# microsoft/ptgnn

Hardware: AMD Instinct MI355X
Metric: edges/sec per MP layer (higher is better)
Workload: dtype f32; 1 GPU; cfg3: Graph2Class-style batch, 48 graphs N=115772, T0=8->T=17, E=625130 (incl. reverse+self), Typilus GGNN arch: 8 GGNN layers H=128 (+concat residual), max; hidden=128, mode=forward (inference), fp32, plan_build_in_step=True, message_rows=shared per (edge type, source) pair, parallelism=single GPU, minibatches_rotated=4

## Files before the change

ptgnn_amd/csrc/stream_gemm.hip:

```cpp
#include <stdlib.h>

#include "dense_common.h"
#include <atomic>

#include "stream_gemm.h"

namespace ptgnn_amd {
namespace {

using u32x4 = __attribute__((ext_vector_type(4))) uint32_t;

constexpr int kLdsBudget = 160 * 1024;
constexpr size_t kEpiBytes = 16 + 8 * 8 * 36 * sizeof(float);

__device__ __forceinline__ f32x16 zero16() {
  f32x16 v;
#pragma unroll
  for (int r = 0; r < 16; ++r) v[r] = 0.f;
  return v;
}

struct ARows {
  const float *c0, *c1, *n0, *n1;
};

__device__ __forceinline__ float4 load_piece(const ARows &r, int cc, int ch0, int nch, int g) {
  const bool nx = cc >= nch;
  const int c = nx ? cc - nch : cc;
  const float *b0 = nx ? r.n0 : r.c0;
  const float *b1 = nx ? r.n1 : r.c1;
  const float *p = c < ch0 ? b0 + c * 32 : b1 + (c - ch0) * 32;
  return *reinterpret_cast<const float4 *>(p + g * 8);
}

__device__ __forceinline__ int lane_piece_offset(int hi) { return hi * 4; }

template <int NBLK, int NACC, int PH, bool GRU>
__device__ __forceinline__ void chunk_f32(f32x16 (&acc)[NACC], float4 (&buf)[4], float4 (&bcur)[NBLK],
                                          const float *bl, int cbs, int kofs, int kofs_next, const ARows &rows,
                                          int cnext, int ch0, int nch) {
#pragma unroll
  for (int g = 0; g < 4; ++g) {
    float4 bn[NBLK];
    const int ko = g < 3 ? kofs + (g + 1) * 8 : kofs_next;
#pragma unroll
    for (int n = 0; n < NBLK; ++n) bn[n] = *reinterpret_cast<const float4 *>(bl + n * cbs + ko);
    __builtin_amdgcn_sched_barrier(0);
    const float4 a = buf[g];
#define PTGNN_STEP(C)                                                                     \
    _Pragma("unroll") for (int n = 0; n < NBLK; ++n) {                                    \
      const int t = (GRU && PH == 1 && n == 2) ? 3 : n;                                   \
      acc[t] = __builtin_amdgcn_mfma_f32_32x32x2f32(a.C, bcur[n].C, acc[t], 0, 0, 0);     \
    }
    PTGNN_STEP(x) PTGNN_STEP(y) PTGNN_STEP(z) PTGNN_STEP(w)
#undef PTGNN_STEP
    __builtin_amdgcn_sched_barrier(0);
#pragma unroll
    for (int n = 0; n < NBLK; ++n) bcur[n] = bn[n];
  }
#pragma unroll
  for (int g = 0; g < 4; ++g) {
    buf[g] = load_piece(rows, cnext, ch0, nch, g);
    __builtin_amdgcn_sched_barrier(0);
  }
}

struct Slab {
  int ld;
  __device__ __forceinline__ Slab(int K, int ) { ld = K + 4; }
  static size_t bytes(int K, int rows) { return (size_t)rows * (K + 4) * 4; }

  __device__ __forceinline__ void put4(float *smem, int r, int k, float4 v) const {
    *reinterpret_cast<float4 *>(smem + r * ld + k) = v;
  }
};

template <int NT, typename SrcFn, typename LiveFn>
__device__ __forceinline__ void fill_slab(float *smem, const Slab &sl, int rows, int kq, SrcFn src, LiveFn live) {
  constexpr int UB = 8;
  const int total = rows * kq;
  for (int i0 = threadIdx.x; i0 < total; i0 += NT * UB) {
    float4 v[UB];
    int rr[UB], qq[UB];
#pragma unroll
    for (int u = 0; u < UB; ++u) {
      const int i = i0 + u * NT;
      const int ic = i < total ? i : total - 1;
      rr[u] = ic / kq;
      qq[u] = ic - rr[u] * kq;
    }
#pragma unroll
    for (int u = 0; u < UB; ++u) {
      v[u] = *reinterpret_cast<const float4 *>(src(rr[u], qq[u]));
      __builtin_amdgcn_sched_barrier(0);
    }
#pragma unroll
    for (int u = 0; u < UB; ++u) {
      if (i0 + u * NT < total) sl.put4(smem, rr[u], qq[u] * 4, live(rr[u]) ? v[u] : make_float4(0.f, 0.f, 0.f, 0.f));
    }
  }
}

template <int NBLK, int NACC, bool GRU>
__device__ __forceinline__ void unit_kloop(f32x16 (&acc)[NACC], float4 (&a0)[4], float4 (&a1)[4],
                                           const float *smem, const Slab &sl, int li, int hi,
                                           const ARows &rows, int ch0, int nch) {
  const float *bl = smem + li * sl.ld + hi * 4;
  const int cbs = 32 * sl.ld;
  const int e0 = GRU ? ch0 : nch;
  float4 bcur[NBLK];
#pragma unroll
  for (int n = 0; n < NBLK; ++n) bcur[n] = *reinterpret_cast<const float4 *>(bl + n * cbs);
  for (int c = 0; c < e0; c += 2) {
    const int kn = c + 2 < nch ? c * 32 + 64 : 0;
    chunk_f32<NBLK, NACC, 0, GRU>(acc, a0, bcur, bl, cbs, c * 32, c * 32 + 32, rows, c + 2, ch0, nch);
    chunk_f32<NBLK, NACC, 0, GRU>(acc, a1, bcur, bl, cbs, c * 32 + 32, kn, rows, c + 3, ch0, nch);
  }
  if constexpr (GRU) {
    for (int c = ch0; c < nch; c += 2) {
      const int kn = c + 2 < nch ? c * 32 + 64 : 0;
      chunk_f32<NBLK, NACC, 1, GRU>(acc, a0, bcur, bl, cbs, c * 32, c * 32 + 32, rows, c + 2, ch0, nch);
      chunk_f32<NBLK, NACC, 1, GRU>(acc, a1, bcur, bl, cbs, c * 32 + 32, kn, rows, c + 3, ch0, nch);
    }
  }
}

__device__ __forceinline__ void prologue_loads(float4 (&a0)[4], float4 (&a1)[4], const ARows &rows, int ch0,
                                               int nch) {
#pragma unroll
  for (int g = 0; g < 4; ++g) {
    a0[g] = load_piece(rows, 0, ch0, nch, g);
    __builtin_amdgcn_sched_barrier(0);
  }
#pragma unroll
  for (int g = 0; g < 4; ++g) {
    a1[g] = load_piece(rows, 1, ch0, nch, g);
    __builtin_amdgcn_sched_barrier(0);
  }
}

__device__ __forceinline__ void unit_fence() {
  __builtin_amdgcn_s_waitcnt(0x0F70);
  __builtin_amdgcn_sched_barrier(0);
}

__device__ __forceinline__ int claim_unit(int *counter) {
  int v = 0;
  if ((threadIdx.x & 63) == 0) v = atomicAdd(counter, 1);
  return __builtin_amdgcn_readfirstlane(v);
}

constexpr int kTqLd = 36;
constexpr int kTqFloats = 8 * kTqLd;

__device__ __forceinline__ float4 tq_transpose(float *tq, int lane, int li, int hi, float v0, float v1, float v2,
                                               float v3) {
  float *w = tq + (4 * hi) * kTqLd + li;
  w[0] = v0; w[kTqLd] = v1; w[2 * kTqLd] = v2; w[3 * kTqLd] = v3;
  __builtin_amdgcn_wave_barrier();
  const float4 o = *reinterpret_cast<const float4 *>(tq + (lane >> 3) * kTqLd + (lane & 7) * 4);
  __builtin_amdgcn_wave_barrier();
  return o;
}

__device__ __forceinline__ void tq_untranspose(float *tq, int lane, int li, int hi, float4 in, float (&v)[4]) {
  *reinterpret_cast<float4 *>(tq + (lane >> 3) * kTqLd + (lane & 7) * 4) = in;
  __builtin_amdgcn_wave_barrier();
  const float *r = tq + (4 * hi) * kTqLd + li;
  v[0] = r[0]; v[1] = r[kTqLd]; v[2] = r[2 * kTqLd]; v[3] = r[3 * kTqLd];
  __builtin_amdgcn_wave_barrier();
}

using u32x4 = __attribute__((ext_vector_type(4))) uint32_t;

__device__ __forceinline__ __amdgpu_buffer_rsrc_t rows_descriptor(float *base , int64_t ld, int64_t rows_left,
                                                                  int width ) {
  const uint64_t b = reinterpret_cast<uint64_t>(base);
  const uint32_t lo = __builtin_amdgcn_readfirstlane((uint32_t)b), hi = __builtin_amdgcn_readfirstlane((uint32_t)(b >> 32));
  const int64_t rows = rows_left < 32 ? rows_left : 32;
  const int64_t bytes = rows > 0 ? ((rows - 1) * ld + width) * 4 : 0;
  return __builtin_amdgcn_make_buffer_rsrc(reinterpret_cast<float *>(((uint64_t)hi << 32) | lo), 0,
                                           __builtin_amdgcn_readfirstlane((int)bytes), 0x00020000);
}

__device__ __forceinline__ void store_row4(__amdgpu_buffer_rsrc_t rsrc, int lane_bytes, int uniform_bytes, float4 o) {
  const u32x4 v = {__float_as_uint(o.x), __float_as_uint(o.y), __float_as_uint(o.z), __float_as_uint(o.w)};
  __builtin_amdgcn_raw_buffer_store_b128(v, rsrc, lane_bytes + uniform_bytes, 0, 0);
}

template <int ACT, bool BIAS = true>
__device__ __forceinline__ void store_block_tq(const f32x16 &c, float *tq, float *yblk ,
                                               int64_t ld_y, float bv, int64_t rows_left, int lane, int li, int hi,
                                               const float *addblk = nullptr, int64_t ld_add = 0) {
  auto val = [&](int r) { return BIAS ? act_apply<ACT>(c[r] + bv) : act_apply<ACT>(c[r]); };
  float4 addv[4];
  if (addblk) {
#pragma unroll
    for (int q = 0; q < 4; ++q) {
      int64_t r = 8 * q + (lane >> 3);
      r = r < rows_left ? r : rows_left - 1;
      addv[q] = *reinterpret_cast<const float4 *>(addblk + r * ld_add + (lane & 7) * 4);
    }
  }
#ifdef PTGNN_GLOBAL_STORES
  float *yp = yblk + (int64_t)(lane >> 3) * ld_y + (lane & 7) * 4;
#pragma unroll
  for (int q = 0; q < 4; ++q) {
    float4 o = tq_transpose(tq, lane, li, hi, val(4 * q), val(4 * q + 1), val(4 * q + 2), val(4 * q + 3));
    if (addblk) { o.x += addv[q].x; o.y += addv[q].y; o.z += addv[q].z; o.w += addv[q].w; }
    if (8 * q + (lane >> 3) < rows_left) *reinterpret_cast<float4 *>(yp + (int64_t)(8 * q) * ld_y) = o;
  }
#else
  const __amdgpu_buffer_rsrc_t rsrc = rows_descriptor(yblk, ld_y, rows_left, 32);
  const int ldb = (int)ld_y * 4;
  const int lane_bytes = (lane >> 3) * ldb + (lane & 7) * 16;
#pragma unroll
  for (int q = 0; q < 4; ++q) {
    float4 o = tq_transpose(tq, lane, li, hi, val(4 * q), val(4 * q + 1), val(4 * q + 2), val(4 * q + 3));
    if (addblk) { o.x += addv[q].x; o.y += addv[q].y; o.z += addv[q].z; o.w += addv[q].w; }
    store_row4(rsrc, lane_bytes, 8 * q * ldb, o);
  }
#endif
}

struct LinearArgs {
  const float *x; int64_t rows; int K; int64_t ld_x;
  const float *w; int n_out; const float *bias; int act;
  float *y; int64_t ld_y;
  const float *addend; int64_t ld_add;
  int nrb, ncs, rps, run_len;
  int lds_floats;
  int vec_store;
};

template <int ACT>
__device__ __forceinline__ void store_block(const f32x16 &c, float *yp, int64_t ld_y, float bv, int64_t row0,
                                            int64_t rows, int hi) {
  if (row0 + 32 <= rows) {
#pragma unroll
    for (int r = 0; r < 16; ++r)
      yp[(int64_t)((r & 3) + 8 * (r >> 2)) * ld_y] = act_apply<ACT>(c[r] + bv);
  } else {
#pragma unroll
    for (int r = 0; r < 16; ++r) {
      const int rr = (r & 3) + 8 * (r >> 2);
      if (row0 + rr + 4 * hi < rows) yp[(int64_t)rr * ld_y] = act_apply<ACT>(c[r] + bv);
    }
  }
}

template <int NB>
__device__ __forceinline__ void linear_epilogue(const LinearArgs &p, f32x16 (&acc)[NB], float *tq, int64_t row0,
                                                int col_base, int lane, int li, int hi) {
#pragma unroll
  for (int n = 0; n < NB; ++n) {
    const int col = col_base + n * 32 + li;
    if (col_base + n * 32 < p.n_out) {
      const float bv = p.bias ? p.bias[col] : 0.f;
      if (p.vec_store) {
        float *yb = p.y + row0 * p.ld_y + col_base + n * 32;
        const int64_t left = p.rows - row0;
        if (p.bias) {
#pragma unroll
          for (int r = 0; r < 16; ++r) acc[n][r] += bv;
        }
        const float *ab = p.addend ? p.addend + row0 * p.ld_add + col_base + n * 32 : nullptr;
        if (p.act == PTGNN_AMD_ACT_TANH) store_block_tq<PTGNN_AMD_ACT_TANH, false>(acc[n], tq, yb, p.ld_y, 0.f, left, lane, li, hi, ab, p.ld_add);
        else if (p.act == PTGNN_AMD_ACT_RELU) store_block_tq<PTGNN_AMD_ACT_RELU, false>(acc[n], tq, yb, p.ld_y, 0.f, left, lane, li, hi, ab, p.ld_add);
        else store_block_tq<PTGNN_AMD_ACT_NONE, false>(acc[n], tq, yb, p.ld_y, 0.f, left, lane, li, hi, ab, p.ld_add);
      } else {
        float *yp = p.y + (row0 + 4 * hi) * p.ld_y + col;
        if (p.act == PTGNN_AMD_ACT_TANH) store_block<PTGNN_AMD_ACT_TANH>(acc[n], yp, p.ld_y, bv, row0, p.rows, hi);
        else if (p.act == PTGNN_AMD_ACT_RELU) store_block<PTGNN_AMD_ACT_RELU>(acc[n], yp, p.ld_y, bv, row0, p.rows, hi);
        else store_block<PTGNN_AMD_ACT_NONE>(acc[n], yp, p.ld_y, bv, row0, p.rows, hi);
      }
    }
    acc[n] = zero16();
  }
}

template <int NB>
__global__ __launch_bounds__(512, 2) void k_stream_linear(LinearArgs p) {
  extern __shared__ __attribute__((aligned(16))) float smem[];
  constexpr int NT = 512, BN = 32 * NB;
  const int b = blockIdx.x, G = gridDim.x;
  int slab, part;
  if (G % (kNumXcd * p.ncs) == 0) {
    const int xcd = b % kNumXcd, j = b / kNumXcd;
    slab = j % p.ncs;
    part = xcd + kNumXcd * (j / p.ncs);
  } else {
    slab = b / p.rps;
    part = b % p.rps;
  }
  const int rb0 = part * p.run_len;
  const int rb1 = rb0 + p.run_len < p.nrb ? rb0 + p.run_len : p.nrb;
  if (rb0 >= rb1) return;
  const int count = rb1 - rb0;

  const Slab sl(p.K, BN);
  int *counter = reinterpret_cast<int *>(smem + p.lds_floats);
  float *const tq = smem + p.lds_floats + 4 + (threadIdx.x >> 6) * kTqFloats;
  if (threadIdx.x == 0) *counter = 0;
  const int col_base = slab * BN;
  fill_slab<NT>(smem, sl, BN, p.K >> 2,
                       [&](int r, int q) {
                         const int wr = col_base + r < p.n_out ? col_base + r : p.n_out - 1;
                         return p.w + (int64_t)wr * p.K + q * 4;
                       },
                       [&](int r) { return col_base + r < p.n_out; });
  __syncthreads();

  const int lane = threadIdx.x & 63;
  const int li = lane & 31, hi = lane >> 5;
  const int nch = p.K >> 5;
  const int lofs = lane_piece_offset(hi);
  auto rowp = [&](int u) {
    int64_t row = (int64_t)(rb0 + (u < count ? u : count - 1)) * 32 + li;
    row = row < p.rows ? row : p.rows - 1;
    return p.x + row * p.ld_x + lofs;
  };
  int cur = claim_unit(counter);
  if (cur >= count) return;
  int nxt = claim_unit(counter);
  ARows rows;
  rows.c0 = rows.c1 = rowp(cur);
  rows.n0 = rows.n1 = rowp(nxt);
  float4 a0[4], a1[4];
  prologue_loads(a0, a1, rows, nch, nch);
  f32x16 acc[NB];
#pragma unroll
  for (int n = 0; n < NB; ++n) acc[n] = zero16();

  while (cur < count) {
    const int nn = claim_unit(counter);
    unit_fence();
    unit_kloop<NB, NB, false>(acc, a0, a1, smem, sl, li, hi, rows, nch, nch);
    const int64_t row0 = (int64_t)(rb0 + cur) * 32;
    linear_epilogue<NB>(p, acc, tq, row0, col_base, lane, li, hi);
    cur = nxt;
    nxt = nn;
    rows.c0 = rows.c1 = rows.n0;
    rows.n0 = rows.n1 = rowp(nxt);
  }
}

struct GruArgs {
  const float *a; int64_t ld_a; const float *h; int64_t ld_h;
  const float *w_ih, *w_hh, *b_ih, *b_hh;
  int64_t n; int M, H;
  float *out; int64_t ld_out; float *gates;
  int nrb, ncs, rps, run_len;
  int lds_floats;
};

__device__ __forceinline__ float fast_sigmoid(float v) {
  return __builtin_amdgcn_rcpf(1.0f + __builtin_amdgcn_exp2f(-1.4426950408889634f * v));
}

using f32x2 = __attribute__((ext_vector_type(2))) float;
__device__ __forceinline__ f32x2 splat2(float v) { return f32x2{v, v}; }
__device__ __forceinline__ f32x2 rcp_1_plus_exp2(f32x2 t) {
  const f32x2 d = f32x2{__builtin_amdgcn_exp2f(t.x), __builtin_amdgcn_exp2f(t.y)} + splat2(1.0f);
  return f32x2{__builtin_amdgcn_rcpf(d.x), __builtin_amdgcn_rcpf(d.y)};
}

__device__ __forceinline__ void gru_epilogue(const GruArgs &p, const f32x16 (&acc)[4], float *tq, int64_t row0,
                                             int j0, int lane, int li, int hi, float bir, float biz, float bin,
                                             float bhr, float bhz, float bhn) {
  const int trow = lane >> 3, tcol = (lane & 7) * 4;
#ifndef PTGNN_GLOBAL_STORES
  const __amdgpu_buffer_rsrc_t out_rsrc = rows_descriptor(p.out + row0 * p.ld_out + j0, p.ld_out, p.n - row0, 32);
  const __amdgpu_buffer_rsrc_t gate_rsrc =
      rows_descriptor(p.gates ? p.gates + row0 * (int64_t)(4 * p.H) + j0 : p.out, 4 * (int64_t)p.H, p.n - row0, 3 * p.H + 32);
#endif
#pragma unroll
  for (int q = 0; q < 4; ++q) {
    int64_t hrow = row0 + 8 * q + trow;
    const bool rvalid = hrow < p.n;
    hrow = rvalid ? hrow : p.n - 1;
    float hp[4];
    tq_untranspose(tq, lane, li, hi, *reinterpret_cast<const float4 *>(p.h + hrow * p.ld_h + j0 + tcol), hp);
    float res[4], rg[4], zg[4], ng[4], hn[4];
    {
#pragma clang fp contract(off)
#pragma unroll
      for (int i = 0; i < 4; i += 2) {
        const int r = 4 * q + i;
        const f32x2 ar = {acc[0][r], acc[0][r + 1]}, az = {acc[1][r], acc[1][r + 1]};
        const f32x2 an = {acc[2][r], acc[2][r + 1]}, ah = {acc[3][r], acc[3][r + 1]};
        const f32x2 hp2 = {hp[i], hp[i + 1]};
        const f32x2 r2 = rcp_1_plus_exp2(((ar + splat2(bir)) + splat2(bhr)) * splat2(-1.4426950408889634f));
        const f32x2 z2 = rcp_1_plus_exp2(((az + splat2(biz)) + splat2(bhz)) * splat2(-1.4426950408889634f));
        const f32x2 h2 = ah + splat2(bhn);
        const f32x2 pre = (an + splat2(bin)) + r2 * h2;
        const f32x2 n2 = splat2(2.0f) * rcp_1_plus_exp2(pre * splat2(-2.8853900817779268f)) - splat2(1.0f);
        const f32x2 o2 = (splat2(1.0f) - z2) * n2 + z2 * hp2;
        rg[i] = r2.x; rg[i + 1] = r2.y; zg[i] = z2.x; zg[i + 1] = z2.y; hn[i] = h2.x; hn[i + 1] = h2.y;
        ng[i] = n2.x; ng[i + 1] = n2.y; res[i] = o2.x; res[i + 1] = o2.y;
      }
    }
    const float4 o = tq_transpose(tq, lane, li, hi, res[0], res[1], res[2], res[3]);
#ifdef PTGNN_GLOBAL_STORES
    if (rvalid) *reinterpret_cast<float4 *>(p.out + hrow * p.ld_out + j0 + tcol) = o;
#else
    store_row4(out_rsrc, trow * (int)p.ld_out * 4 + tcol * 4, 8 * q * (int)p.ld_out * 4, o);
#endif
    if (p.gates) {
      const float4 o_r = tq_transpose(tq, lane, li, hi, rg[0], rg[1], rg[2], rg[3]);
      const float4 o_z = tq_transpose(tq, lane, li, hi, zg[0], zg[1], zg[2], zg[3]);
      const float4 o_n = tq_transpose(tq, lane, li, hi, ng[0], ng[1], ng[2], ng[3]);
      const float4 o_h = tq_transpose(tq, lane, li, hi, hn[0], hn[1], hn[2], hn[3]);
#ifdef PTGNN_GLOBAL_STORES
      float *gp = p.gates + hrow * (int64_t)(4 * p.H) + j0 + tcol;
      if (rvalid) {
        *reinterpret_cast<float4 *>(gp) = o_r;
        *reinterpret_cast<float4 *>(gp + p.H) = o_z;
        *reinterpret_cast<float4 *>(gp + 2 * p.H) = o_n;
        *reinterpret_cast<float4 *>(gp + 3 * p.H) = o_h;
      }
#else
      const int gl = trow * 16 * p.H + tcol * 4, gu = 8 * q * 16 * p.H;
      store_row4(gate_rsrc, gl, gu, o_r);
      store_row4(gate_rsrc, gl, gu + 4 * p.H, o_z);
      store_row4(gate_rsrc, gl, gu + 8 * p.H, o_n);
      store_row4(gate_rsrc, gl, gu + 12 * p.H, o_h);
#endif
    }
  }
}

__global__ __launch_bounds__(512, 2) void k_stream_gru(GruArgs p) {
  extern __shared__ __attribute__((aligned(16))) float smem[];
  constexpr int NT = 512;
  const int b = blockIdx.x, G = gridDim.x;
  int slab, part;
  if (G % (kNumXcd * p.ncs) == 0) {
    const int xcd = b % kNumXcd, j = b / kNumXcd;
    slab = j % p.ncs;
    part = xcd + kNumXcd * (j / p.ncs);
  } else {
    slab = b / p.rps;
    part = b % p.rps;
  }
  const int rb0 = part * p.run_len;
  const int rb1 = rb0 + p.run_len < p.nrb ? rb0 + p.run_len : p.nrb;
  if (rb0 >= rb1) return;
  const int count = rb1 - rb0;

  const int K = p.M + p.H;
  const Slab sl(K, 96);
  int *counter = reinterpret_cast<int *>(smem + p.lds_floats);
  float *const tq = smem + p.lds_floats + 4 + (threadIdx.x >> 6) * kTqFloats;
  if (threadIdx.x == 0) *counter = 0;
  const int j0 = slab * 32;
  {
    const int mq = p.M >> 2;
    fill_slab<NT>(smem, sl, 96, K >> 2,
                         [&](int r, int q) {
                           const int gate = r >> 5, jj = j0 + (r & 31);
                           return q < mq ? p.w_ih + ((int64_t)gate * p.H + jj) * p.M + q * 4
                                         : p.w_hh + ((int64_t)gate * p.H + jj) * p.H + (q - mq) * 4;
                         },
                         [](int) { return true; });
  }
  __syncthreads();

  const int lane = threadIdx.x & 63;
  const int li = lane & 31, hi = lane >> 5;
  const int ch0 = p.M >> 5, nch = K >> 5;
  const int lofs = lane_piece_offset(hi);
  auto clampr = [&](int u) {
    const int64_t row = (int64_t)(rb0 + (u < count ? u : count - 1)) * 32 + li;
    return row < p.n ? row : p.n - 1;
  };
  int cur = claim_unit(counter);
  if (cur >= count) return;
  int nxt = claim_unit(counter);
  ARows rows;
  {
    const int64_t r0 = clampr(cur), r1 = clampr(nxt);
    rows.c0 = p.a + r0 * p.ld_a + lofs; rows.c1 = p.h + r0 * p.ld_h + lofs;
    rows.n0 = p.a + r1 * p.ld_a + lofs; rows.n1 = p.h + r1 * p.ld_h + lofs;
  }
  float4 a0[4], a1[4];
  prologue_loads(a0, a1, rows, ch0, nch);
  f32x16 acc[4];
#pragma unroll
  for (int n = 0; n < 4; ++n) acc[n] = zero16();

  const int j = j0 + li;
  const float bir = p.b_ih[j], biz = p.b_ih[p.H + j], bin = p.b_ih[2 * p.H + j];
  const float bhr = p.b_hh[j], bhz = p.b_hh[p.H + j], bhn = p.b_hh[2 * p.H + j];

  while (cur < count) {
    const int nn = claim_unit(counter);
    unit_fence();
    unit_kloop<3, 4, true>(acc, a0, a1, smem, sl, li, hi, rows, ch0, nch);
    gru_epilogue(p, acc, tq, (int64_t)(rb0 + cur) * 32, j0, lane, li, hi, bir, biz, bin, bhr, bhz, bhn);
#pragma unroll
    for (int n = 0; n < 4; ++n) acc[n] = zero16();
    cur = nxt;
    nxt = nn;
    rows.c0 = rows.n0; rows.c1 = rows.n1;
    const int64_t r1 = clampr(nxt);
    rows.n0 = p.a + r1 * p.ld_a + lofs; rows.n1 = p.h + r1 * p.ld_h + lofs;
  }
}

constexpr int kRingPanel = 64;
constexpr int kRingLd = kRingPanel + 4;
constexpr int kRingPanelFloats = 96 * kRingLd;
constexpr int kRingWaves = 4;

__global__ __launch_bounds__(kRingWaves * 64, 2) void k_stream_gru_ring(GruArgs p) {
  extern __shared__ __attribute__((aligned(16))) float smem[];
  const int b = blockIdx.x, G = gridDim.x;
  int slab, part;
  if (G % (kNumXcd * p.ncs) == 0) {
    const int xcd = b % kNumXcd, j = b / kNumXcd;
    slab = j % p.ncs;
    part = xcd + kNumXcd * (j / p.ncs);
  } else {
    slab = b / p.rps;
    part = b % p.rps;
  }
  const int rb0 = part * p.run_len;
  const int rb1 = rb0 + p.run_len < p.nrb ? rb0 + p.run_len : p.nrb;
  if (rb0 >= rb1) return;
  const int count = rb1 - rb0;
  const int rounds = (count + kRingWaves - 1) / kRingWaves;

  const int K = p.M + p.H;
  const int npan = K / kRingPanel;
  const int lane = threadIdx.x & 63, wave = threadIdx.x >> 6;
  const int li = lane & 31, hi = lane >> 5;
  float *const tq = smem + 2 * kRingPanelFloats + wave * kTqFloats;
  const int j0 = slab * 32;
  const int ch0 = p.M >> 5, nch = K >> 5;

  const int trow = threadIdx.x >> 4, tc4 = (threadIdx.x & 15) * 4;
  const int base_ih = (j0 + trow) * p.M + tc4, base_hh = (j0 + trow) * p.H + tc4;
  auto panel_src = [&](int pan, int q) -> const float * {
    const int k0 = pan * kRingPanel;
    const int rq = (q >> 1) * p.H + (q & 1) * 16;
    return k0 < p.M ? p.w_ih + (base_ih + rq * p.M + k0) : p.w_hh + (base_hh + rq * p.H + (k0 - p.M));
  };
  auto panel_dst = [&](int buf, int q) -> float * {
    return smem + buf * kRingPanelFloats + (trow + 16 * q) * kRingLd + tc4;
  };
  {
#pragma unroll
    for (int q = 0; q < 6; ++q) *reinterpret_cast<float4 *>(panel_dst(0, q)) = *reinterpret_cast<const float4 *>(panel_src(0, q));
  }
  __syncthreads();

  const int lofs = lane_piece_offset(hi);
  auto clampr = [&](int u) {
    const int64_t row = (int64_t)(rb0 + (u < count ? u : count - 1)) * 32 + li;
    return row < p.n ? row : p.n - 1;
  };
  ARows rows;
  {
    const int64_t r0 = clampr(wave), r1 = clampr(wave + kRingWaves);
    rows.c0 = p.a + r0 * p.ld_a + lofs; rows.c1 = p.h + r0 * p.ld_h + lofs;
    rows.n0 = p.a + r1 * p.ld_a + lofs; rows.n1 = p.h + r1 * p.ld_h + lofs;
  }
  float4 a0[4], a1[4];
  prologue_loads(a0, a1, rows, ch0, nch);
  f32x16 acc[4];
#pragma unroll
  for (int n = 0; n < 4; ++n) acc[n] = zero16();

  const int j = j0 + li;
  const float bir = p.b_ih[j], biz = p.b_ih[p.H + j], bin = p.b_ih[2 * p.H + j];
  const float bhr = p.b_hh[j], bhz = p.b_hh[p.H + j], bhn = p.b_hh[2 * p.H + j];
  const int cbs = 32 * kRingLd;

  int P = 0;
  for (int i = 0; i < rounds; ++i) {
    const int u = i * kRingWaves + wave;
    unit_fence();
#define PTGNN_RING_PANEL(PH)                                                                                   \
  do {                                                                                                         \
    const float *bl = smem + (P & 1) * kRingPanelFloats + li * kRingLd + hi * 4;                               \
    float *const nb = smem + ((P + 1) & 1) * kRingPanelFloats + trow * kRingLd + tc4;                          \
    const int nextpan = pan + 1 < npan ? pan + 1 : 0;                                                          \
    float4 w0 = *reinterpret_cast<const float4 *>(panel_src(nextpan, 0));                                      \
    float4 w1 = *reinterpret_cast<const float4 *>(panel_src(nextpan, 1));                                      \
    float4 w2 = *reinterpret_cast<const float4 *>(panel_src(nextpan, 2));                                      \
    __builtin_amdgcn_sched_barrier(0);                                                                         \
    float4 bcur[3];                                                                                            \
    _Pragma("unroll") for (int n = 0; n < 3; ++n) bcur[n] = *reinterpret_cast<const float4 *>(bl + n * cbs);   \
    chunk_f32<3, 4, PH, true>(acc, a0, bcur, bl, cbs, 0, 32, rows, 2 * pan + 2, ch0, nch);                     \
    *reinterpret_cast<float4 *>(nb) = w0;                                                                      \
    *reinterpret_cast<float4 *>(nb + 16 * kRingLd) = w1;                                                       \
    *reinterpret_cast<float4 *>(nb + 32 * kRingLd) = w2;                                                       \
    w0 = *reinterpret_cast<const float4 *>(panel_src(nextpan, 3));                                             \
    w1 = *reinterpret_cast<const float4 *>(panel_src(nextpan, 4));                                             \
    w2 = *reinterpret_cast<const float4 *>(panel_src(nextpan, 5));                                             \
    __builtin_amdgcn_sched_barrier(0);                                                                         \
    chunk_f32<3, 4, PH, true>(acc, a1, bcur, bl, cbs, 32, 0, rows, 2 * pan + 3, ch0, nch);                     \
    *reinterpret_cast<float4 *>(nb + 48 * kRingLd) = w0;                                                       \
    *reinterpret_cast<float4 *>(nb + 64 * kRingLd) = w1;                                                       \
    *reinterpret_cast<float4 *>(nb + 80 * kRingLd) = w2;                                                       \
    lds_barrier();                              \
  } while (0)
    int pan = 0;
    for (; pan < (ch0 >> 1); ++pan, ++P) PTGNN_RING_PANEL(0);
    for (; pan < npan; ++pan, ++P) PTGNN_RING_PANEL(1);
#undef PTGNN_RING_PANEL
    if (u < count) gru_epilogue(p, acc, tq, (int64_t)(rb0 + u) * 32, j0, lane, li, hi, bir, biz, bin, bhr, bhz, bhn);
#pragma unroll
    for (int n = 0; n < 4; ++n) acc[n] = zero16();
    rows.c0 = rows.n0; rows.c1 = rows.n1;
    const int64_t r1 = clampr(u + 2 * kRingWaves);
    rows.n0 = p.a + r1 * p.ld_a + lofs; rows.n1 = p.h + r1 * p.ld_h + lofs;
  }
}

constexpr int kLinRingPanelFloats = 128 * kRingLd;

__global__ __launch_bounds__(kRingWaves * 64, 2) void k_stream_linear_ring(LinearArgs p) {
  extern __shared__ __attribute__((aligned(16))) float smem[];
  const int b = blockIdx.x, G = gridDim.x;
  int slab, part;
  if (G % (kNumXcd * p.ncs) == 0) {
    const int xcd = b % kNumXcd, j = b / kNumXcd;
    slab = j % p.ncs;
    part = xcd + kNumXcd * (j / p.ncs);
  } else {
    slab = b / p.rps;
    part = b % p.rps;
  }
  const int rb0 = part * p.run_len;
  const int rb1 = rb0 + p.run_len < p.nrb ? rb0 + p.run_len : p.nrb;
  if (rb0 >= rb1) return;
  const int count = rb1 - rb0;
  const int rounds = (count + kRingWaves - 1) / kRingWaves;

  const int K = p.K;
  const int npan = K / kRingPanel, nch = K >> 5;
  const int lane = threadIdx.x & 63, wave = threadIdx.x >> 6;
  const int li = lane & 31, hi = lane >> 5;
  float *const tq = smem + 2 * kLinRingPanelFloats + wave * kTqFloats;
  const int col_base = slab * 128;

  const int trow = threadIdx.x >> 4, tc4 = (threadIdx.x & 15) * 4;
  const int wbase = (col_base + trow) * K + tc4;
  const int wq = 16 * K;
  {
    float *const d = smem + trow * kRingLd + tc4;
#pragma unroll
    for (int q = 0; q < 8; ++q)
      *reinterpret_cast<float4 *>(d + 16 * q * kRingLd) = *reinterpret_cast<const float4 *>(p.w + (wbase + q * wq));
  }
  __syncthreads();

  const int lofs = lane_piece_offset(hi);
// ... 403 lines not shown
                o.x = keep_scaled(o.x, m, 0, q.scale); o.y = keep_scaled(o.y, m, 1, q.scale);
                o.z = keep_scaled(o.z, m, 2, q.scale); o.w = keep_scaled(o.w, m, 3, q.scale);
              }
#ifdef PTGNN_GLOBAL_STORES
              *reinterpret_cast<float4 *>(yr + n * 32) = o;
#else
              store_row4(msg_rsrc, srow * ldb + (scol + n * 32) * 4, 8 * r * ldb, o);
#endif
              __builtin_amdgcn_sched_barrier(0);
            }
          }
#pragma unroll
          for (int n = 0; n < NB; ++n) acc[n] = zero16();
        }
        if (nxt >= count) break;
        cur = nxt; nxt = n2;
        c0 = n0; c1 = n1;
        if constexpr (DROP == 1) mc = mn;
      }
    }
    u = seg_end;
  }
}

std::atomic<int> g_mode{-1};

bool debug_on() {
  static int v = -1;
  if (v < 0) v = getenv("PTGNN_AMD_DEBUG") ? 1 : 0;
  return v == 1;
}

template <typename Kern>
bool set_lds(Kern kern, size_t bytes) {
  const char *why = "";
  if (raise_dynamic_lds(kern, bytes, &why)) return true;
  if (debug_on()) fprintf(stderr, "[ptgnn_amd] stream kernel: %zu B of LDS refused (%s) -> tile kernel\n", bytes, why);
  return false;
}

void dense_runs(int nrb, int ncs, int &rps, int &run_len, int max_wg = 0) {
  if (max_wg <= 0) max_wg = num_compute_units();
  rps = max_wg / ncs;
  if (rps < 1) rps = 1;
  if (rps >= kNumXcd && (rps / kNumXcd * kNumXcd) * ncs * 10 >= max_wg * 9) rps = rps / kNumXcd * kNumXcd;
  if (rps > nrb) rps = nrb;
  run_len = (nrb + rps - 1) / rps;
  rps = (nrb + run_len - 1) / run_len;
}

}

int stream_gemm_mode() {
  int mode = g_mode.load(std::memory_order_relaxed);
  if (mode < 0) {
    const char *e = getenv("PTGNN_AMD_GEMM");
    const int m = e ? atoi(e) : 1;
    mode = (m == 0 || m == 1) ? m : 1;
    g_mode.store(mode, std::memory_order_relaxed);
  }
  return mode;
}

void stream_gemm_set_mode(int mode) { g_mode.store(mode, std::memory_order_relaxed); }

#define PTGNN_STREAM_DISPATCH_NB(NBV, KERN, ...)     \
  switch (NBV) {                                      \
    case 1: KERN(1, __VA_ARGS__); break;              \
    case 2: KERN(2, __VA_ARGS__); break;              \
    case 3: KERN(3, __VA_ARGS__); break;              \
    default: KERN(4, __VA_ARGS__); break;             \
  }

int stream_linear(const float *x, int64_t rows, int32_t k, int64_t ld_x, const float *w, int32_t n_out,
                  const float *bias, int act, float *y, int64_t ld_y, hipStream_t st, const float *addend,
                  int64_t ld_add) {
  const int mode = stream_gemm_mode();
  if (mode == 0) return 0;
  if (addend && (ld_y % 4 != 0 || !aligned16(y) || ld_add % 4 != 0 || !aligned16(addend))) return 0;
  if (k % 64 != 0 || n_out % 32 != 0 || ld_x % 4 != 0 || !aligned16(x) || !aligned16(w)) return 0;
  if (rows >= ((int64_t)1 << 31) * 32) return 0;
  int bn = n_out >= 128 ? 128 : n_out;
  {
    const bool fits128 = Slab::bytes(k, 128) + kEpiBytes <= (size_t)kLdsBudget;
    const bool fits64 = Slab::bytes(k, 64) + kEpiBytes <= (size_t)kLdsBudget;
    const char *bn_env = getenv("PTGNN_AMD_LINEAR_BN");
    const int want = bn_env ? atoi(bn_env) : 0;
    const char *ring_force = getenv("PTGNN_AMD_LINEAR_RING");
    const bool ring_forced = ring_force && ring_force[0] == '1';
    if (!ring_forced && n_out % 128 == 0 && n_out <= 256 && fits64 && (want == 64 || (want != 128 && !fits128))) bn = 64;
  }
  const int nb = bn / 32;
  const char *ring_env = getenv("PTGNN_AMD_LINEAR_RING");
  const bool force_ring = ring_env && ring_env[0] == '1', no_ring = ring_env && ring_env[0] == '0';
  const char *force = getenv("PTGNN_AMD_FORCE_STREAM");
  const bool forced = force && force[0] == '1';
  const bool ring_shape = n_out % 128 == 0 && (int64_t)n_out * k < ((int64_t)1 << 30) && (rows >= 32 * 64 || forced);
  const bool ring = ring_shape && (force_ring || (!no_ring && Slab::bytes(k, bn) + kEpiBytes > (size_t)kLdsBudget));
  if (!ring) {
    const int64_t units = (rows + 31) / 32 * ((n_out + bn - 1) / bn);
    if (!forced && (units < (int64_t)num_compute_units() * 8 * 3 || (n_out + bn - 1) / bn > 4)) return 0;
  }
  const size_t slab = Slab::bytes(k, bn);
  const size_t lds = slab + 16 + 8 * kTqFloats * sizeof(float);
  LinearArgs p;
  p.x = x; p.rows = rows; p.K = k; p.ld_x = ld_x; p.w = w; p.n_out = n_out; p.bias = bias; p.act = act;
  p.y = y; p.ld_y = ld_y; p.addend = addend; p.ld_add = ld_add;
  p.nrb = (int)((rows + 31) / 32);
  p.ncs = (n_out + bn - 1) / bn;
  p.vec_store = (ld_y % 4 == 0 && aligned16(y)) ? 1 : 0;
  if (ring) {
    const size_t rlds = (size_t)(2 * kLinRingPanelFloats + kRingWaves * kTqFloats) * sizeof(float);
    dense_runs(p.nrb, p.ncs, p.rps, p.run_len, 2 * num_compute_units());
    p.lds_floats = 0;
    auto kern = k_stream_linear_ring;
    if (!set_lds(kern, rlds)) return 0;
    kern<<<(unsigned)(p.ncs * p.rps), kRingWaves * 64, rlds, st>>>(p);
    count_launch(PTGNN_AMD_KERNEL_STREAM_LINEAR_RING);
    return 1;
  }
  if (lds > (size_t)kLdsBudget) return 0;
  dense_runs(p.nrb, p.ncs, p.rps, p.run_len);
  p.lds_floats = (int)(slab / 4);
  const unsigned grid = (unsigned)(p.ncs * p.rps);
#define PTGNN_K(NBV, UNUSED)                                                        \
  do {                                                                              \
    auto kern = k_stream_linear<NBV>;                                               \
    if (!set_lds(kern, lds)) return 0;                                              \
    kern<<<grid, 512, lds, st>>>(p);                                                \
  } while (0)
  PTGNN_STREAM_DISPATCH_NB(nb, PTGNN_K, 0);
#undef PTGNN_K
  count_launch(PTGNN_AMD_KERNEL_STREAM_LINEAR);
  return 1;
}

int stream_gru(const float *a, int64_t ld_a, const float *h, int64_t ld_h, const float *w_ih,
               const float *w_hh, const float *b_ih, const float *b_hh, int64_t n, int32_t m, int32_t hd,
               float *out, int64_t ld_out, float *gates, hipStream_t st) {
  const int mode = stream_gemm_mode();
  if (mode == 0) return 0;
  if (m % 64 != 0 || hd % 64 != 0 || ld_a % 4 != 0 || ld_h % 4 != 0 || ld_out % 4 != 0 || !aligned16(a) ||
      !aligned16(h) || !aligned16(out) || (gates && !aligned16(gates)) || !aligned16(w_ih) || !aligned16(w_hh))
    return 0;
  if (n >= ((int64_t)1 << 31) * 32) return 0;
  const int K = m + hd;
  const size_t slab = Slab::bytes(K, 96);
  const size_t lds = slab + 16 + 8 * kTqFloats * sizeof(float);
  GruArgs p;
  p.a = a; p.ld_a = ld_a; p.h = h; p.ld_h = ld_h; p.w_ih = w_ih; p.w_hh = w_hh; p.b_ih = b_ih; p.b_hh = b_hh;
  p.n = n; p.M = m; p.H = hd; p.out = out; p.ld_out = ld_out; p.gates = gates;
  p.nrb = (int)((n + 31) / 32);
  p.ncs = hd / 32;
  const char *ring_env = getenv("PTGNN_AMD_GRU_RING");
  const bool force_ring = ring_env && ring_env[0] == '1';
  if ((lds > (size_t)kLdsBudget && !(ring_env && ring_env[0] == '0')) || force_ring) {
    const size_t rlds = (size_t)(2 * kRingPanelFloats + kRingWaves * kTqFloats) * sizeof(float);
    dense_runs(p.nrb, p.ncs, p.rps, p.run_len, 2 * num_compute_units());
    p.lds_floats = 0;
    auto kern = k_stream_gru_ring;
    if (!set_lds(kern, rlds)) return 0;
    kern<<<(unsigned)(p.ncs * p.rps), kRingWaves * 64, rlds, st>>>(p);
    count_launch(PTGNN_AMD_KERNEL_STREAM_GRU_RING);
    return 1;
  }
  if (lds > (size_t)kLdsBudget) return 0;
  dense_runs(p.nrb, p.ncs, p.rps, p.run_len);
  p.lds_floats = (int)(slab / 4);
  const unsigned grid = (unsigned)(p.ncs * p.rps);
  {
    auto kern = k_stream_gru;
    if (!set_lds(kern, lds)) return 0;
    kern<<<grid, 512, lds, st>>>(p);
  }
  count_launch(PTGNN_AMD_KERNEL_STREAM_GRU);
  return 1;
}

static bool edge_v2_shape(int32_t state_dim, int32_t msg_dim, int use_dst, int act) {
  if (stream_gemm_mode() != 1 || act != PTGNN_AMD_ACT_NONE || use_dst) return false;
  const int K = state_dim;
  if (!(K == 64 || K == 128 || K == 256)) return false;
  if (!(msg_dim == 64 || msg_dim == 128)) return false;
  return Slab::bytes(K, msg_dim) + kEpiBytes <= (size_t)kLdsBudget;
}

template <int DROP>
static int edge_v2_launch(const EdgeV2Args &q, int K, int msg_dim, unsigned grid, size_t lds, hipStream_t st) {
#define PTGNN_K(NBV, NCHV)                                            \
  do {                                                                \
    auto kern = k_stream_edge_v2<NBV, NCHV, DROP, 0>;                 \
    if (!set_lds(kern, lds)) return 0;                                \
    kern<<<grid, 512, lds, st>>>(q);                                  \
    count_launch(PTGNN_AMD_KERNEL_STREAM_EDGE_V2);                    \
    return 1;                                                         \
  } while (0)
  if (msg_dim == 128) {
    if (K == 64) PTGNN_K(4, 2);
    if (K == 128) PTGNN_K(4, 4);
    if (K == 256) PTGNN_K(4, 8);
  } else {
    if (K == 64) PTGNN_K(2, 2);
    if (K == 128) PTGNN_K(2, 4);
    if (K == 256) PTGNN_K(2, 8);
  }
#undef PTGNN_K
  return 0;
}

constexpr size_t kEdgeEpiBytes = 16 + (size_t)kEdgeWaves * kTqFloats * sizeof(float);

static int edge_plan(int32_t state_dim, int32_t msg_dim, int use_dst, size_t *slab_bytes) {
  const int mode = stream_gemm_mode();
  if (mode == 0) return 0;
  const int K = use_dst ? 2 * state_dim : state_dim;
  if (K % 64 != 0 || state_dim % 32 != 0 || msg_dim % 32 != 0 || msg_dim > 128) return 0;
  if (Slab::bytes(K, msg_dim) + kEdgeEpiBytes <= (size_t)kLdsBudget) {
    *slab_bytes = Slab::bytes(K, msg_dim);
    return 1;
  }
  return 0;
}

int stream_edge_supported(int32_t state_dim, int32_t msg_dim, int use_dst) {
  size_t b;
  return edge_plan(state_dim, msg_dim, use_dst, &b) != 0;
}

int stream_edge_masked_supported(int32_t state_dim, int32_t msg_dim) {
  return edge_v2_shape(state_dim, msg_dim, 0, PTGNN_AMD_ACT_NONE) ? 1 : 0;
}

int stream_edge(const StreamEdgeTable &tab, const float *x, int64_t ld_x, int64_t num_rows, int32_t state_dim,
                int use_dst, int32_t msg_dim, int act, float *msg, int64_t ld_msg, int64_t msg_row_base,
                hipStream_t st, const StreamEdgeMask *mask) {
  size_t slab = 0;
  const int kind = edge_plan(state_dim, msg_dim, use_dst, &slab);
  const bool v2 = edge_v2_shape(state_dim, msg_dim, use_dst, act);
  if (mask && mask->mode != 0 && !v2) return 0;
  if (kind == 0) return 0;
  const int nb = msg_dim / 32;
  const size_t lds = slab + 16 + kEdgeWaves * kTqFloats * sizeof(float);
  const int total = tab.unit_off[tab.num_types];
  if (total == 0) return 1;
  EdgeArgs p;
  p.tab = tab; p.tab_dev = nullptr; p.x = x; p.ld_x = ld_x; p.H = state_dim; p.use_dst = use_dst; p.M = msg_dim; p.act = act;
  p.msg = msg; p.ld_msg = ld_msg; p.msg_row_base = msg_row_base; p.num_rows = num_rows;
  int budget = num_compute_units();
  if (budget > total / 8 + 1) budget = total / 8 + 1;
  int w[kStreamMaxTypes], sum = 0, nonempty = 0;
  for (int t = 0; t < tab.num_types; ++t) {
    const int64_t u_t = tab.unit_off[t + 1] - tab.unit_off[t];
    w[t] = u_t == 0 ? 0 : (int)(u_t * budget / total);
    if (u_t > 0 && w[t] == 0) w[t] = 1;
    sum += w[t];
    nonempty += u_t > 0;
  }
  if (budget < nonempty) budget = nonempty;
  while (sum != budget) {
    int best = -1;
    double best_v = 0.0;
    for (int t = 0; t < tab.num_types; ++t) {
      const double u_t = (double)(tab.unit_off[t + 1] - tab.unit_off[t]);
      if (u_t == 0) continue;
      if (sum < budget) {
        const double v = u_t / w[t];
        if (best < 0 || v > best_v) { best = t; best_v = v; }
      } else if (w[t] > 1) {
        const double v = u_t / (w[t] - 1);
        if (best < 0 || v < best_v) { best = t; best_v = v; }
      }
    }
    if (best < 0) break;
    w[best] += sum < budget ? 1 : -1;
    sum += sum < budget ? 1 : -1;
  }
  p.tab.wg_off[0] = 0;
  for (int t = 0; t < tab.num_types; ++t) p.tab.wg_off[t + 1] = p.tab.wg_off[t] + w[t];
  for (int t = tab.num_types + 1; t <= kStreamMaxTypes; ++t) {
    p.tab.wg_off[t] = p.tab.wg_off[tab.num_types];
    p.tab.unit_off[t] = p.tab.unit_off[tab.num_types];
  }
  p.run_len = 0;
  p.lds_floats = (int)(slab / 4);
  const unsigned grid = (unsigned)p.tab.wg_off[tab.num_types];
  if (mask && mask->mode != 0) {
    EdgeV2Args q;
    q.e = p;
    q.mask = mask->bits; q.mask_ld = mask->ld; q.mask_col0 = mask->col0; q.scale = mask->scale;
    return mask->mode == 1 ? edge_v2_launch<1>(q, state_dim, msg_dim, grid, lds, st)
                           : edge_v2_launch<2>(q, state_dim, msg_dim, grid, lds, st);
  }
#define PTGNN_K(NBV, UNUSED)                                  \
  do {                                                        \
    auto kern = k_stream_edge<NBV, false>;                    \
    if (!set_lds(kern, lds)) return 0;                        \
    kern<<<grid, kEdgeWaves * 64, lds, st>>>(p);              \
  } while (0)
  PTGNN_STREAM_DISPATCH_NB(nb, PTGNN_K, 0);
#undef PTGNN_K
  count_launch(PTGNN_AMD_KERNEL_STREAM_EDGE);
  return 1;
}

int stream_edge_indirect(const StreamEdgeTable *tab_dev, const float *const *w_per_type, int num_types, const float *x,
                         int64_t ld_x, int64_t num_rows, int32_t state_dim, int32_t msg_dim, int act, float *msg,
                         int64_t ld_msg, hipStream_t st) {
  if (num_types > kStreamMaxTypes) return 0;
  size_t slab = 0;
  const int kind = edge_plan(state_dim, msg_dim, 0, &slab);
  if (kind == 0) return 0;
  const int nb = msg_dim / 32;
  const size_t lds = slab + 16 + kEdgeWaves * kTqFloats * sizeof(float);
  EdgeArgs p;
  p.tab.num_types = num_types;
  for (int t = 0; t < num_types; ++t) p.tab.w[t] = w_per_type[t];
  p.tab_dev = tab_dev;
  p.x = x; p.ld_x = ld_x; p.H = state_dim; p.use_dst = 0; p.M = msg_dim; p.act = act;
  p.msg = msg; p.ld_msg = ld_msg; p.msg_row_base = 0; p.num_rows = num_rows;
  p.run_len = 0;
  p.lds_floats = (int)(slab / 4);
  const unsigned grid = (unsigned)edge_table_budget();
#define PTGNN_K(NBV, UNUSED)                                  \
  do {                                                        \
    auto kern = k_stream_edge<NBV, true>;                     \
    if (!set_lds(kern, lds)) return 0;                        \
// ... 27 lines not shown
```

Measured before the change: 1.326 billion edges/s.

## Split tail GRU row-blocks across waves by gate group with LDS exchange

When a block's unit count is not a multiple of 8 waves, the leftover tail units are split into three sub-tasks per unit: r gate, z gate, and the n gates. Two waves park r/z accumulators in LDS and signal with workgroup-scope atomics, and a third wave waits, combines them and runs the GRU epilogue. This is meant to cut the load imbalance where a few waves do the last full units while the rest sit idle. It costs extra LDS (which may reduce occupancy), spin-waiting, and more sync complexity. It is enabled by default only when gates are not stored.

```diff
diff --git a/ptgnn_amd/csrc/stream_gemm.hip b/ptgnn_amd/csrc/stream_gemm.hip
--- a/ptgnn_amd/csrc/stream_gemm.hip
+++ b/ptgnn_amd/csrc/stream_gemm.hip
@@ -49,7 +49,7 @@
     const float4 a = buf[g];
 #define PTGNN_STEP(C)                                                                     \
     _Pragma("unroll") for (int n = 0; n < NBLK; ++n) {                                    \
-      const int t = (GRU && PH == 1 && n == 2) ? 3 : n;                                   \
+      const int t = (GRU && PH == 1 && n == NBLK - 1) ? NACC - 1 : n;                     \
       acc[t] = __builtin_amdgcn_mfma_f32_32x32x2f32(a.C, bcur[n].C, acc[t], 0, 0, 0);     \
     }
     PTGNN_STEP(x) PTGNN_STEP(y) PTGNN_STEP(z) PTGNN_STEP(w)
@@ -149,6 +149,11 @@
   if ((threadIdx.x & 63) == 0) v = atomicAdd(counter, 1);
   return __builtin_amdgcn_readfirstlane(v);
 }
+
+#ifndef PTGNN_TAIL_SPLIT
+#define PTGNN_TAIL_SPLIT 1
+#endif
+constexpr bool kSplitGru = PTGNN_TAIL_SPLIT != 0;
 
 constexpr int kTqLd = 36;
 constexpr int kTqFloats = 8 * kTqLd;
@@ -352,7 +357,11 @@
   float *out; int64_t ld_out; float *gates;
   int nrb, ncs, rps, run_len;
   int lds_floats;
+  int split;
 };
+
+constexpr int kGruSplitUnits = 6;
+constexpr size_t kGruSplitBytes = (size_t)kGruSplitUnits * 2 * 4096 + 32;
 
 __device__ __forceinline__ float fast_sigmoid(float v) {
   return __builtin_amdgcn_rcpf(1.0f + __builtin_amdgcn_exp2f(-1.4426950408889634f * v));
@@ -452,7 +461,10 @@
   const Slab sl(K, 96);
   int *counter = reinterpret_cast<int *>(smem + p.lds_floats);
   float *const tq = smem + p.lds_floats + 4 + (threadIdx.x >> 6) * kTqFloats;
-  if (threadIdx.x == 0) *counter = 0;
+  float *const xch = smem + p.lds_floats + 4 + 8 * kTqFloats;
+  int *const flags = reinterpret_cast<int *>(xch + kGruSplitUnits * 2048);
+  if (threadIdx.x == 0) counter[0] = counter[1] = 0;
+  if (kSplitGru && p.split && threadIdx.x < 8) flags[threadIdx.x] = 0;
   const int j0 = slab * 32;
   {
     const int mq = p.M >> 2;
@@ -474,37 +486,86 @@
     const int64_t row = (int64_t)(rb0 + (u < count ? u : count - 1)) * 32 + li;
     return row < p.n ? row : p.n - 1;
   };
-  int cur = claim_unit(counter);
-  if (cur >= count) return;
-  int nxt = claim_unit(counter);
-  ARows rows;
-  {
-    const int64_t r0 = clampr(cur), r1 = clampr(nxt);
-    rows.c0 = p.a + r0 * p.ld_a + lofs; rows.c1 = p.h + r0 * p.ld_h + lofs;
-    rows.n0 = p.a + r1 * p.ld_a + lofs; rows.n1 = p.h + r1 * p.ld_h + lofs;
-  }
-  float4 a0[4], a1[4];
-  prologue_loads(a0, a1, rows, ch0, nch);
-  f32x16 acc[4];
-#pragma unroll
-  for (int n = 0; n < 4; ++n) acc[n] = zero16();
-
+  int tail = kSplitGru && p.split ? count & 7 : 0;
+  if (tail > kGruSplitUnits) tail = 0;
+  const int whole = count - tail;
   const int j = j0 + li;
   const float bir = p.b_ih[j], biz = p.b_ih[p.H + j], bin = p.b_ih[2 * p.H + j];
   const float bhr = p.b_hh[j], bhz = p.b_hh[p.H + j], bhn = p.b_hh[2 * p.H + j];
 
-  while (cur < count) {
-    const int nn = claim_unit(counter);
-    unit_fence();
-    unit_kloop<3, 4, true>(acc, a0, a1, smem, sl, li, hi, rows, ch0, nch);
-    gru_epilogue(p, acc, tq, (int64_t)(rb0 + cur) * 32, j0, lane, li, hi, bir, biz, bin, bhr, bhz, bhn);
+  int cur = claim_unit(counter);
+  if (cur < whole) {
+    int nxt = claim_unit(counter);
+    ARows rows;
+    {
+      const int64_t r0 = clampr(cur), r1 = clampr(nxt);
+      rows.c0 = p.a + r0 * p.ld_a + lofs; rows.c1 = p.h + r0 * p.ld_h + lofs;
+      rows.n0 = p.a + r1 * p.ld_a + lofs; rows.n1 = p.h + r1 * p.ld_h + lofs;
+    }
+    float4 a0[4], a1[4];
+    prologue_loads(a0, a1, rows, ch0, nch);
+    f32x16 acc[4];
 #pragma unroll
     for (int n = 0; n < 4; ++n) acc[n] = zero16();
-    cur = nxt;
-    nxt = nn;
-    rows.c0 = rows.n0; rows.c1 = rows.n1;
-    const int64_t r1 = clampr(nxt);
-    rows.n0 = p.a + r1 * p.ld_a + lofs; rows.n1 = p.h + r1 * p.ld_h + lofs;
+
+    while (cur < whole) {
+      const int nn = claim_unit(counter);
+      unit_fence();
+      unit_kloop<3, 4, true>(acc, a0, a1, smem, sl, li, hi, rows, ch0, nch);
+      gru_epilogue(p, acc, tq, (int64_t)(rb0 + cur) * 32, j0, lane, li, hi, bir, biz, bin, bhr, bhz, bhn);
+#pragma unroll
+      for (int n = 0; n < 4; ++n) acc[n] = zero16();
+      cur = nxt;
+      nxt = nn;
+      rows.c0 = rows.n0; rows.c1 = rows.n1;
+      const int64_t r1 = clampr(nxt);
+      rows.n0 = p.a + r1 * p.ld_a + lofs; rows.n1 = p.h + r1 * p.ld_h + lofs;
+    }
+  }
+  if (tail > 0) {
+    const int nsub = 3 * tail;
+    int s = claim_unit(counter + 1);
+    if (s >= nsub) return;
+    const int cbs = 32 * sl.ld;
+    auto rows_of = [&](int q, const float *&ra, const float *&rh) {
+      const int64_t r = clampr(whole + (q < nsub ? q : nsub - 1) / 3);
+      ra = p.a + r * p.ld_a + lofs; rh = p.h + r * p.ld_h + lofs;
+    };
+    ARows rows;
+    rows_of(s, rows.c0, rows.c1);
+    rows_of(s + 8, rows.n0, rows.n1);
+    float4 a0[4], a1[4];
+    prologue_loads(a0, a1, rows, ch0, nch);
+    for (; s < nsub; s += 8) {
+      const int unit = s / 3, grp = s - unit * 3;
+      float4 *const park = reinterpret_cast<float4 *>(xch) + (unit * 2) * 256 + lane;
+      unit_fence();
+      if (grp < 2) {
+        f32x16 acc[1] = {zero16()};
+        unit_kloop<1, 1, false>(acc, a0, a1, smem + grp * cbs, sl, li, hi, rows, ch0, nch);
+#pragma unroll
+        for (int q = 0; q < 4; ++q)
+          park[grp * 256 + q * 64] = make_float4(acc[0][4 * q], acc[0][4 * q + 1], acc[0][4 * q + 2], acc[0][4 * q + 3]);
+        if (lane == 0) __hip_atomic_fetch_add(flags + unit, 1, __ATOMIC_RELEASE, __HIP_MEMORY_SCOPE_WORKGROUP);
+      } else {
+        f32x16 nh[2] = {zero16(), zero16()};
+        unit_kloop<1, 2, true>(nh, a0, a1, smem + 2 * cbs, sl, li, hi, rows, ch0, nch);
+        while (__hip_atomic_load(flags + unit, __ATOMIC_ACQUIRE, __HIP_MEMORY_SCOPE_WORKGROUP) < 2) __builtin_amdgcn_s_sleep(1);
+        f32x16 acc[4];
+#pragma unroll
+        for (int g = 0; g < 2; ++g) {
+#pragma unroll
+          for (int q = 0; q < 4; ++q) {
+            const float4 v = park[g * 256 + q * 64];
+            acc[g][4 * q] = v.x; acc[g][4 * q + 1] = v.y; acc[g][4 * q + 2] = v.z; acc[g][4 * q + 3] = v.w;
+          }
+        }
+        acc[2] = nh[0]; acc[3] = nh[1];
+        gru_epilogue(p, acc, tq, (int64_t)(rb0 + whole + unit) * 32, j0, lane, li, hi, bir, biz, bin, bhr, bhz, bhn);
+      }
+      rows.c0 = rows.n0; rows.c1 = rows.n1;
+      rows_of(s + 16, rows.n0, rows.n1);
+    }
   }
 }
 
@@ -1214,6 +1275,7 @@
   p.n = n; p.M = m; p.H = hd; p.out = out; p.ld_out = ld_out; p.gates = gates;
   p.nrb = (int)((n + 31) / 32);
   p.ncs = hd / 32;
+  p.split = 0;
   const char *ring_env = getenv("PTGNN_AMD_GRU_RING");
   const bool force_ring = ring_env && ring_env[0] == '1';
   if ((lds > (size_t)kLdsBudget && !(ring_env && ring_env[0] == '0')) || force_ring) {
@@ -1229,11 +1291,13 @@
   if (lds > (size_t)kLdsBudget) return 0;
   dense_runs(p.nrb, p.ncs, p.rps, p.run_len);
   p.lds_floats = (int)(slab / 4);
+  p.split = (kSplitGru && !gates && lds + kGruSplitBytes <= (size_t)kLdsBudget) ? 1 : 0;
+  const size_t lds_launch = p.split ? lds + kGruSplitBytes : lds;
   const unsigned grid = (unsigned)(p.ncs * p.rps);
   {
     auto kern = k_stream_gru;
-    if (!set_lds(kern, lds)) return 0;
-    kern<<<grid, 512, lds, st>>>(p);
+    if (!set_lds(kern, lds_launch)) return 0;
+    kern<<<grid, 512, lds_launch, st>>>(p);
   }
   count_launch(PTGNN_AMD_KERNEL_STREAM_GRU);
   return 1;
```

After: 1.343 billion edges/s, median of 6. +1.3%, better.
